# saifahmadgit/go2-sim2real-locomotion-rl

Hardware: AMD Instinct MI355X
Metric: env-steps/sec (all envs) Go2 walk 4096 envs; 1/2/4/8-GPU scaling (higher is better)
Workload: dtype f32

## Files before the change

go2_sim2real_locomotion_rl_amd/csrc/go2sim.hip:

```cpp

#include <hip/hip_runtime.h>

#include <algorithm>
#include <cstddef>
#include <cstdint>
#include <cstdio>
#include <cstdlib>
#include <cstring>
#include <new>
#include <vector>

#include "../../include/go2sim.h"
#include "../../include/go2sim_detmath.h"

#define DEV __device__ __forceinline__
#define DEVN __device__ __noinline__

namespace {

constexpr int NL = GO2SIM_NL, ND = GO2SIM_ND, NQ = GO2SIM_NQ, NG = GO2SIM_NG, NJ = GO2SIM_NJ;
constexpr int NPAIR = GO2SIM_NPAIR_MAX, MAXC = GO2SIM_MAX_CONTACTS, MAXB = GO2SIM_MAX_BROAD, MAXR = GO2SIM_MAX_ROWS;
constexpr int JOINT_FIXED = 0, JOINT_REVOLUTE = 1, JOINT_FREE = 4;
constexpr int GEOM_PLANE = 0, GEOM_SPHERE = 1, GEOM_CYLINDER = 3, GEOM_BOX = 5, GEOM_TERRAIN = 7;
constexpr int TERRAIN_CB = 4;
// ... 851 lines not shown
  xl2 = v2 * iv.z; xl1 = __builtin_fmaf(-lv.z, xl2, v1) * iv.y; xl0 = __builtin_fmaf(-lv.x, xl1, __builtin_fmaf(-lv.y, xl2, v0)) * iv.x;
#pragma unroll
  for (int k = 0; k < 6; ++k) xb[k] = x[k];
}
#endif
struct DynData {
  float cinr_I[NL * 9], cinr_pos[NL * 3], cinr_mass[NL];
  float crb_I[NL * 9], crb_pos[NL * 3], crb_mass[NL];
  float cdof_ang[ND * 3], cdof_vel[ND * 3], cdofd_ang[ND * 3], cdofd_vel[ND * 3];
  float cd_vel[NL * 3], cd_ang[NL * 3], cdd_vel[NL * 3], cdd_ang[NL * 3], cfrc_vel[NL * 3], cfrc_ang[NL * 3];
  float f_ang[ND * 3], f_vel[ND * 3];
  float vel[ND], qf_applied[ND], qf_passive[ND], force[ND], out[ND], Dinv[ND];
  float M[ND * ND], L[ND * ND];
  int ctrl_mode[ND];
};
#if GO2SIM_FAST_ORDER
static_assert(!ARROW_SHAPE || (offsetof(DynData, Dinv) % 8 == 0 && sizeof(DynData) % 8 == 0), "arrow_solve reads DynData::Dinv with 8-byte LDS loads");
#endif

template <int T>
DEV void tk_stage_links(const E& e, KinData* s, int tl) {
  team_for<NL, T>(tl, [&](int i_l) { st3(s->l_pos, i_l, e.l_pos()[i_l]); st4(s->l_quat, i_l, e.l_quat()[i_l]); });
}
template <int T, class MT>
DEV void tk_kinematics(const MT& m, const E& e, KinData* s, int tl, bool force_update_fixed, DynData* dk = nullptr) {
  PH_BEGIN
  const bool legs = (T == 32 || T == 64) && m.leg_form;
  if (legs) {
    const int r = m.leg_root;
    const int rq = m.joints[m.links[r].joint_start].q_start;
    const V3 rpos = v3(s->qpos[rq], s->qpos[rq + 1], s->qpos[rq + 2]);
    Q4 rquat = q4(s->qpos[rq + 3], s->qpos[rq + 4], s->qpos[rq + 5], s->qpos[rq + 6]);
    const float rn = dm_sqrt(norm_sqr(rquat));
    rquat = q4(rquat.w / rn, rquat.x / rn, rquat.y / rn, rquat.z / rn);
    if (tl == 0) {
      const auto& L = m.links[r];
      const int i_j = L.joint_start, ds = m.joints[i_j].dof_start;
      st3(s->xanchor, i_j, rpos);
      st3(s->xaxis, i_j, v3(0, 0, 1));
      gstore(e, FO(dof_pos), ds + 0, rpos.x); gstore(e, FO(dof_pos), ds + 1, rpos.y); gstore(e, FO(dof_pos), ds + 2, rpos.z);
      if (dk) { dk->out[ds] = rpos.x; dk->out[ds + 1] = rpos.y; dk->out[ds + 2] = rpos.z; }
      st3(s->l_pos, r, rpos); st4(s->l_quat, r, rquat); e.l_pos()[r] = rpos; e.l_quat()[r] = rquat;
    }
    Q4 ql = q4(0, 0, 0, 0);
    if (tl < LEG_K * LEG_D) {
      const Joint& J = m.joints[m.links[m.leg_links[tl]].joint_start];
      const float dp = s->qpos[J.q_start] - m.qpos0[J.q_start];
      gstore(e, FO(dof_pos), J.dof_start, dp);
// ... 56 lines not shown
          pos = pos_; quat = quat_;
          gstore(e, FO(dof_pos), dof_start + 0, pos.x); gstore(e, FO(dof_pos), dof_start + 1, pos.y); gstore(e, FO(dof_pos), dof_start + 2, pos.z);
          if (dk) { dk->out[dof_start] = pos.x; dk->out[dof_start + 1] = pos.y; dk->out[dof_start + 2] = pos.z; }
        } else if (J.type == JOINT_REVOLUTE) {
          V3 axis = m.dofs[dof_start].motion_ang;
          V3 anchor = transform_by_quat(J.pos, quat) + pos;
          st3(s->xanchor, i_j, anchor);
          st3(s->xaxis, i_j, transform_by_quat(axis, quat));
          float dp = s->qpos[q_start] - m.qpos0[q_start];
          gstore(e, FO(dof_pos), dof_start, dp);
          if (dk) dk->out[dof_start] = dp;
          Q4 qloc = rotvec_to_quat(axis * dp, m.eps);
          quat = transform_quat_by_quat(qloc, quat);
          pos = anchor - transform_by_quat(J.pos, quat);
        }
      }
      if (!(L.parent == -1 && L.is_fixed)) { st3(s->l_pos, i_l, pos); st4(s->l_quat, i_l, quat); e.l_pos()[i_l] = pos; e.l_quat()[i_l] = quat; }
    }
    team_sync();
  }
  PH(18)
  for (int i_l = tl; i_l < NL; i_l += T) {
    const auto& L = m.links[i_l];
    s->mass[i_l] = L.mass + gload(e, FO(mass_shift), i_l);
    V3 ipbw; Q4 iq;
    transform_pos_quat_by_trans_quat(L.inertial_pos + (V3)e.com_shift()[i_l], L.inertial_quat, ld3(s->l_pos, i_l), ld4(s->l_quat, i_l), ipbw, iq);
    st3(s->i_pos, i_l, ipbw); st4(s->i_quat, i_l, iq);
  }
  team_sync();
  V3 rc[2];
#pragma unroll
  for (int i_e = 0; i_e < 2; ++i_e) {
    const Entity& en = m.entities[i_e];
    V3 root_com_bw = v3(0, 0, 0); float mass_sum = 0.0f;
    for (int i_l = en.link_start; i_l < en.link_end; ++i_l) {
      float mass = s->mass[i_l];
      mass_sum = mass_sum + mass;
      root_com_bw = root_com_bw + mass * ld3(s->i_pos, i_l);
    }
    rc[i_e] = root_com_bw / mass_sum;
  }
  team_sync();
  for (int i_l = tl; i_l < NL; i_l += T) {
    const auto& L = m.links[i_l];
    V3 r = (L.entity == 0) ? rc[0] : rc[1];
    e.root_com()[i_l] = r;
    V3 ip = ld3(s->i_pos, i_l) - r;
    Q4 iq = ld4(s->i_quat, i_l);
    if (!dk) e.i_pos()[i_l] = ip;
// ... 187 lines not shown
    atomicOr(&e.err()[0], GO2SIM_ERR_INVALID_ACC_NAN);
  }
  team_sync();
}

template <int T>
DEV void integrate_fk_body(const Pool& P, const ModelS* __restrict__ mp, int b, KinData* lds, char* ms_raw, bool pre, float pre_vel, float pre_acc) {
  const ModelS& ms = *(const ModelS*)ms_raw;
  wg_dma_to_lds<(int)sizeof(ModelS)>(ms_raw, mp);
  const int tl = threadIdx.x % T, slot = threadIdx.x / T;
  const ModelView m(&ms, mp);
  E e(P, b < P.B ? b : P.B - 1);
  KinData* s = &lds[slot];
  PH_BEGIN
  if (pre) { if (tl < ND) { s->vel[tl] = pre_vel; s->vel_next[tl] = pre_acc; } }
  else {
    team_stage<ND, T>(tl, [&](int d) { return gload(e, FO(vel), d); }, [&](int d, float v) { s->vel[d] = v; });
    team_stage<ND, T>(tl, [&](int d) { return aload(e, AO(acc), d); }, [&](int d, float a) { s->vel_next[d] = a; });
  }
  team_stage<NQ, T>(tl, [&](int q) { return gload(e, FO(qpos), q); }, [&](int q, float v) { s->qpos[q] = v; });
  team_for<ND, T>(tl, [&](int d) { s->vel_next[d] = s->vel[d] + s->vel_next[d] * m.substep_dt; });
  if (tl == 0) s->valid = 1;
  tk_stage_links<T>(e, s, tl);
  team_sync();
  if (b >= P.B) return;
  tk_integrate<T>(m, e, s, tl);
  PH(40)
  tk_kinematics<T>(m, e, s, tl, false);
  PH(41)
}
template <int T>
__global__ __launch_bounds__(64) void k_integrate_fk_team(Pool P, const ModelS* __restrict__ mp) {
  STAMP(STK_INT_FK)
  constexpr int EPW = 64 / T;
  __shared__ KinData lds[EPW];
  __shared__ alignas(16) char ms_raw[MODELS_LDS_BYTES];
  integrate_fk_body<T>(P, mp, xcd_block() * EPW + (int)threadIdx.x / T, lds, ms_raw, false, 0.0f, 0.0f);
}

template <int T>
__global__ __launch_bounds__(64) void k_fk_team(Pool P, const ModelS* __restrict__ mp, int force_update_fixed, const int* __restrict__ cond) {
  constexpr int EPW = 64 / T;
  __shared__ KinData lds[EPW];
  __shared__ alignas(16) char ms_raw[MODELS_LDS_BYTES];
  const ModelS& ms = *(const ModelS*)ms_raw;
  if (cond && *cond <= 0) return;
  wg_dma_to_lds<(int)sizeof(ModelS)>(ms_raw, mp);
  const int tl = threadIdx.x % T, slot = threadIdx.x / T;
  const int b = xcd_block() * EPW + slot;
  const ModelView m(&ms, mp);
  E e(P, b < P.B ? b : P.B - 1);
  KinData* s = &lds[slot];
  team_stage<ND, T>(tl, [&](int d) { return gload(e, FO(vel), d); }, [&](int d, float v) { s->vel[d] = v; });
  team_stage<NQ, T>(tl, [&](int q) { return gload(e, FO(qpos), q); }, [&](int q, float v) { s->qpos[q] = v; });
  tk_stage_links<T>(e, s, tl);
  team_sync();
  if (b >= P.B) return;
  tk_kinematics<T>(m, e, s, tl, force_update_fixed != 0);
}

template <int T, class MT>
DEV void tk_dynamics(const MT& m, const E& e, DynData* s, int tl, bool env_valid) {
  PH_BEGIN
  const bool legs = (T == 32 || T == 64) && m.leg_form;
  if (legs) {
    for (int c = tl; c < 13; c += T) {
      auto at = [&](int i_l) -> float* { return (c < 9) ? &s->crb_I[9 * i_l + c] : ((c < 12) ? &s->crb_pos[3 * i_l + c - 9] : &s->crb_mass[i_l]); };
      const int r = m.leg_root;
      float x[LEG_K][LEG_D];
#pragma unroll
      for (int l = 0; l < LEG_K; ++l)
#pragma unroll
        for (int d = 0; d < LEG_D; ++d) x[l][d] = *at(m.leg_links[LEG_D * l + d]);
      float a = *at(r);
#pragma unroll
      for (int l = 0; l < LEG_K; ++l) {
#pragma unroll
        for (int d = LEG_D - 2; d >= 0; --d) { x[l][d] = x[l][d] + x[l][d + 1]; *at(m.leg_links[LEG_D * l + d]) = x[l][d]; }
      }
#pragma unroll
      for (int l = 0; l < LEG_K; ++l) a = a + x[l][0];
      *at(r) = a;
    }
    team_sync();
  }
// ... 201 lines not shown
  for (int lev = (legs ? -1 : m.n_levels - 2); lev >= 0; --lev) {
    int n_par = m.level_start[lev + 1] - m.level_start[lev];
    for (int w = tl; w < n_par * 6; w += T) {
      int i_p = m.level_links[m.level_start[lev] + w / 6], comp = w % 6;
      float* dst = (comp < 3) ? &s->cfrc_vel[3 * i_p + comp] : &s->cfrc_ang[3 * i_p + comp - 3];
      float a = *dst;
      for (int c = m.child_start[i_p]; c < m.child_start[i_p + 1]; ++c) {
        int i_l = m.child_list[c];
        a = a + ((comp < 3) ? s->cfrc_vel[3 * i_l + comp] : s->cfrc_ang[3 * i_l + comp - 3]);
      }
      *dst = a;
    }
    team_sync();
  }
  for (int i_d = tl; i_d < ND; i_d += T) {
    int i_l = m.dof_link[i_d];
    float qf_bias = dot(ld3(s->cdof_ang, i_d), ld3(s->cfrc_ang, i_l)) + dot(ld3(s->cdof_vel, i_d), ld3(s->cfrc_vel, i_l));
    float f = s->qf_passive[i_d] - qf_bias + s->qf_applied[i_d];
    s->force[i_d] = f;
    if (env_valid) { astore(e, AO(force), i_d, f); astore(e, AO(qf_smooth), i_d, f); }
  }
  team_sync();
  PH(24)
  bool solved = false;
#if GO2SIM_FAST_ORDER
  if constexpr (T == 32 || T == 64) {
    if (arrow) {
      const int leg = (tl >> 3) & 3, u = tl & 7, ub = u < 6 ? u : 5;
      const int p0 = dm_arrow_dof(m.arrow_mode, leg, 0), p1 = dm_arrow_dof(m.arrow_mode, leg, 1), p2 = dm_arrow_dof(m.arrow_mode, leg, 2);
      float xb[6], x0, x1, x2;
      arrow_solve<T>(AF, s->force[p0], s->force[p1], s->force[p2], s->force[ub], s->Dinv, tl, xb, x0, x1, x2);
      if (tl == 0) {
#pragma unroll
        for (int k = 0; k < 6; ++k) s->out[k] = xb[k];
      }
      if (tl < 32 && u == 0) { s->out[p0] = x0; s->out[p1] = x1; s->out[p2] = x2; }
      solved = true;
    }
  }
#endif
  if (!solved) {
    float y[ND];
#pragma unroll
    for (int i_d_ = 0; i_d_ < ND; ++i_d_) {
      const int i_d = ND - i_d_ - 1;
      float cur = s->force[i_d];
// ... 28 lines not shown
}
template <int T>
struct BroadData {
  alignas(16) float amin[NG * 4], amax[NG * 4];
  alignas(16) unsigned long long skey[2 * NG];
  alignas(8) int rank_mm[NG * 2];
  int cand_key[MAXB], cand_pair[MAXB];
  unsigned pair_sorted[MAXB];
};
static_assert(NPAIR <= (1 << 16) && NG <= (1 << 8), "broad_word: 8 bits per geom, 16 bits of pair index");
DEV unsigned broad_word(int packed, int pidx) { return (unsigned)packed | ((unsigned)pidx << 16); }
constexpr int BROAD_PAD = 12;
template <int T> constexpr bool BROAD_OVERLAY = sizeof(BroadData<T>) + BROAD_PAD <= sizeof(DynData);
template <bool OVERLAY, int T> struct BroadSeparate { BroadData<T> k[64 / T]; DEV BroadData<T>* at(int slot, DynData*) { return &k[slot]; } };
template <int T> struct BroadSeparate<true, T> {
  DEV BroadData<T>* at(int slot, DynData* d) {
    static_assert(sizeof(BroadData<T>) + BROAD_PAD <= sizeof(DynData) && sizeof(DynData) % 4 == 0 && alignof(BroadData<T>) == 16, "BroadData overlay");
    return (BroadData<T>*)((char*)d + (16 - (slot * (int)sizeof(DynData)) % 16) % 16);
  }
};
static_assert((BROAD_OVERLAY<16> && BROAD_OVERLAY<32> && BROAD_OVERLAY<64>) || NG != 28 || ND != 18, "the Go2 shape keeps the dynamics kernels' LDS size");

template <int T>
DEV void tk_broadphase(const Model& m, const E& e, BroadData<T>* s, int tl) {
  const float inf = dm_bits2f(0x7f800000u);
  PH_BEGIN
  const int nc_old = e.n_contacts()[0];
  const bool first = e.first_time()[0] != 0;
  const unsigned ncv_old = (unsigned)e.ncache_valid()[tl < NCV ? tl : NCV - 1];
  constexpr int n2 = 2 * NG, NK = (2 * NG + T - 1) / T, NPI = (NPAIR + T - 1) / T, NGR = (NG + T - 1) / T;
  int sig_[NK];
#pragma unroll
  for (int q = 0; q < NK; ++q) { const int i = tl + q * T; sig_[q] = e.sort_ig()[i < n2 ? i : n2 - 1]; }
  int packed_[NPI];
  {
    const int n_pairs = m.n_pairs;
#pragma unroll
    for (int it = 0; it < NPI; ++it) { int pidx = it * T + tl; int v = m.pair_list[pidx < NPAIR ? pidx : NPAIR - 1]; packed_[it] = (pidx < n_pairs) ? v : -1; }
  }
  V3 lower_[NGR], upper_[NGR];
#pragma unroll
  for (int g = 0; g < NGR; ++g) {
    const int i_g = (g * T + tl < NG) ? g * T + tl : NG - 1;
    V3 lower = v3(inf, inf, inf), upper = v3(-inf, -inf, -inf);
    V3 gp = e.g_pos()[i_g]; Q4 gq = e.g_quat()[i_g];
#pragma unroll
    for (int c = 0; c < 8; ++c) {
      V3 corner = transform_by_trans_quat(m.geoms[i_g].aabb[c], gp, gq);
      lower = vmin(lower, corner); upper = vmax(upper, corner);
    }
    lower_[g] = lower; upper_[g] = upper;
  }
  team_sync();
#pragma unroll
  for (int g = 0; g < NGR; ++g) {
    const int i_g = (g * T + tl < NG) ? g * T + tl : NG - 1;
    *(float4*)&s->amin[4 * i_g] = make_float4(lower_[g].x, lower_[g].y, lower_[g].z, 0.0f);
    *(float4*)&s->amax[4 * i_g] = make_float4(upper_[g].x, upper_[g].y, upper_[g].z, 0.0f);
  }
  team_sync();
  PH(30)
  int r[NK]; float sorted_v[NK]; int sorted_sg[NK];
  unsigned long long key[NK];
#pragma unroll
  for (int q = 0; q < NK; ++q) {
    const int i = (tl + q * T < n2) ? tl + q * T : n2 - 1;
    const int sg = first ? ((i >> 1) | ((i & 1) ? 0x100 : 0)) : sig_[q];
    const int g = sg & 0xff;
    const float v = (sg & 0x100) ? s->amax[4 * g] : s->amin[4 * g];
    unsigned u = (unsigned)__float_as_int(v + 0.0f);
    u = (u & 0x80000000u) ? ~u : (u | 0x80000000u);
// ... 83 lines not shown
  const int tl = threadIdx.x % T, slot = threadIdx.x / T;
  const int b = xcd_block() * EPW + slot;
  const bool env_valid = b < P.B;
  const ModelView m(&ms, mp);
  E e(P, env_valid ? b : P.B - 1);
  DynData* s = &lds[slot];
  PH_BEGIN
  team_stage<NL * 9, T>(tl, [&](int k) { return aload(e, AO(cinr_inertial), k); }, [&](int k, float v) { s->cinr_I[k] = v; s->crb_I[k] = v; });
  team_stage<NL * 3, T>(tl, [&](int k) { return aload(e, AO(cinr_pos), k); }, [&](int k, float v) { s->cinr_pos[k] = v; s->crb_pos[k] = v; });
  team_stage<NL, T>(tl, [&](int k) { return aload(e, AO(cinr_mass), k); }, [&](int k, float v) { s->cinr_mass[k] = v; s->crb_mass[k] = v; });
  team_stage<ND, T>(tl, [&](int d) { return __int_as_float((int)e.ctrl_mode()[d]); }, [&](int d, float v) { s->ctrl_mode[d] = __float_as_int(v); });
  team_stage<ND * 3, T>(tl, [&](int k) { return aload(e, AO(cdof_ang), k); }, [&](int k, float v) { s->cdof_ang[k] = v; });
  team_stage<ND * 3, T>(tl, [&](int k) { return aload(e, AO(cdof_vel), k); }, [&](int k, float v) { s->cdof_vel[k] = v; });
  team_stage<ND * 3, T>(tl, [&](int k) { return aload(e, AO(cdofd_ang), k); }, [&](int k, float v) { s->cdofd_ang[k] = v; });
  team_stage<ND * 3, T>(tl, [&](int k) { return aload(e, AO(cdofd_vel), k); }, [&](int k, float v) { s->cdofd_vel[k] = v; });
  team_stage<ND, T>(tl, [&](int d) { return gload(e, FO(ctrl_force), d); }, [&](int d, float v) { s->qf_applied[d] = v; });
  team_stage<ND, T>(tl, [&](int d) { return gload(e, FO(ctrl_pos), d); }, [&](int d, float v) { s->qf_passive[d] = v; });
  team_stage<ND, T>(tl, [&](int d) { return gload(e, FO(ctrl_vel), d); }, [&](int d, float v) { s->force[d] = v; });
  team_stage<ND, T>(tl, [&](int d) { return gload(e, FO(dof_pos), d); }, [&](int d, float v) { s->out[d] = v; });
  team_stage<NL * 6, T>(tl, [&](int k) { return gload(e, FO(ext), k); },
                        [&](int k, float v) { int i_l = k / 6, c = k % 6; if (c < 3) s->cfrc_ang[3 * i_l + c] = v; else s->cfrc_vel[3 * i_l + c - 3] = v; });
  team_sync();
  PH(20)
  tk_dynamics<T>(m, e, s, tl, env_valid);
  if (env_valid) tk_broadphase<T>(*gm, e, lds_b.at(slot, s), tl);
}


template <bool OVERLAY, int EPW> struct KinSeparate { KinData k[EPW]; DEV KinData* at(int slot, void*) { return &k[slot]; } };
template <int EPW> struct KinSeparate<true, EPW> { DEV KinData* at(int, void* overlay) { return (KinData*)overlay; } };
constexpr bool KIN_OVERLAY = sizeof(KinData) <= 2 * sizeof(float) * ND * ND;
template <int T>
DEV void integrate_fk_dynamics_body(const Pool& P, const ModelS* __restrict__ mp, const Model* __restrict__ gm, int b, DynData* lds_d, char* ms_raw,
                                    KinSeparate<KIN_OVERLAY, 64 / T>& lds_k, BroadSeparate<BROAD_OVERLAY<T>, T>& lds_b, bool pre, float pre_vel, float pre_acc) {
  const ModelS& ms = *(const ModelS*)ms_raw;
  wg_dma_to_lds<(int)sizeof(ModelS)>(ms_raw, mp);
  const int tl = threadIdx.x % T, slot = threadIdx.x / T;
  const ModelView m(&ms, mp);
  asm volatile("" : "+v"(b));
  E e(P, b < P.B ? b : P.B - 1);
  DynData* d = &lds_d[slot];
  static_assert(offsetof(DynData, L) == offsetof(DynData, M) + sizeof(float) * ND * ND, "KinData overlay");
  KinData* s = lds_k.at(slot, d->M);
  PH_BEGIN
  if (pre) { if (tl < ND) { s->vel[tl] = pre_vel; s->vel_next[tl] = pre_acc; } }
  else {
    team_stage<ND, T>(tl, [&](int i) { return gload(e, FO(vel), i); }, [&](int i, float v) { s->vel[i] = v; });
    team_stage<ND, T>(tl, [&](int i) { return aload(e, AO(acc), i); }, [&](int i, float a) { s->vel_next[i] = a; });
  }
  team_stage<NQ, T>(tl, [&](int q) { return gload(e, FO(qpos), q); }, [&](int q, float v) { s->qpos[q] = v; });
  team_stage<ND, T>(tl, [&](int i) { return __int_as_float((int)e.ctrl_mode()[i]); }, [&](int i, float v) { d->ctrl_mode[i] = __float_as_int(v); });
  team_stage<ND, T>(tl, [&](int i) { return gload(e, FO(ctrl_force), i); }, [&](int i, float v) { d->qf_applied[i] = v; });
  team_stage<ND, T>(tl, [&](int i) { return gload(e, FO(ctrl_pos), i); }, [&](int i, float v) { d->qf_passive[i] = v; });
  team_stage<ND, T>(tl, [&](int i) { return gload(e, FO(ctrl_vel), i); }, [&](int i, float v) { d->force[i] = v; });
  team_stage<NL * 6, T>(tl, [&](int k) { return gload(e, FO(ext), k); },
                        [&](int k, float v) { int i_l = k / 6, c = k % 6; if (c < 3) d->cfrc_ang[3 * i_l + c] = v; else d->cfrc_vel[3 * i_l + c - 3] = v; });
  team_for<ND, T>(tl, [&](int i) { s->vel_next[i] = s->vel[i] + s->vel_next[i] * m.substep_dt; });
  if (tl == 0) s->valid = 1;
  tk_stage_links<T>(e, s, tl);
  team_sync();
  if (b >= P.B) return;
  tk_integrate<T>(m, e, s, tl);
  PH(40)
  tk_kinematics<T>(m, e, s, tl, false, d);
  team_for<ND, T>(tl, [&](int i) { d->vel[i] = s->vel[i]; });
  team_sync();
  PH(41)
  tk_dynamics<T>(m, e, d, tl, true);
  tk_broadphase<T>(*gm, e, lds_b.at(slot, d), tl);
}
template <int T>
__global__ __launch_bounds__(64) void k_integrate_fk_dynamics_team(Pool P, const ModelS* __restrict__ mp, const Model* __restrict__ gm) {
  STAMP(STK_INT_FK_DYN)
  constexpr int EPW = 64 / T;
  __shared__ alignas(16) DynData lds_d[EPW];
  __shared__ alignas(16) char ms_raw[MODELS_LDS_BYTES];
  __shared__ KinSeparate<KIN_OVERLAY, EPW> lds_k;
  __shared__ BroadSeparate<BROAD_OVERLAY<T>, T> lds_b;
  integrate_fk_dynamics_body<T>(P, mp, gm, xcd_block() * EPW + (int)threadIdx.x / T, lds_d, ms_raw, lds_k, lds_b, false, 0.0f, 0.0f);
}

DEV int wrap180(float x) {
  if (!(x >= 0.0f)) return 0;
  int i = (x >= 180.0f) ? (int)(x - 180.0f) : (int)x;
  return (i > 179) ? 179 : i;
}
DEV int clampidx(float x) {
  if (!(x >= 0.0f)) return 0;
  return (x >= 179.0f) ? 179 : (int)x;
}
DEV V3 support_cylinder_local(const Model& m, const Geom& G, V3 d_mesh, int* vid_out = nullptr) {
  const float PI = 3.14159265358979323846f;
// ... 1906 lines not shown
        const float active = (float)(rw.Ja < 0.0f);
        const float xs[3] = {rw.q0 * active, rw.q1 * active, rw.q2 * active}, bs[3] = {t0, t1, t2};
        float tot[3];
        team_serial_sum<T, 3>(xs, bs, tl, nseg, tot);
        t0 = tot[0]; t1 = tot[1]; t2 = tot[2];
        done = true;
      }
    }
    if (!done) {
#pragma unroll 16
      for (int c = 0; c < n_con; ++c) {
        float active = (float)(s->Jaref[c] < 0.0f);
        t0 = t0 + s->qf0[c] * active; t1 = t1 + s->qf1[c] * active; t2 = t2 + s->qf2[c] * active;
      }
    }
    p0.alpha = 0.0f; p0.cost = t0; p0.grad = t1; p0.hess = 2.0f * t2;
    if (p0.hess <= 0.0f) p0.hess = m.eps;
  }
  LS_MARK(50)
  return ts_linesearch_tail<T>(m, s, tl, n_con, nseg, rw, gtol, qg0, qg1, qg2, p0);
}

#undef LS_MARK
template <int T, class S, class MT>
DEV int ts_solve(const MT& m, const E& e, S* s, int tl, int nc, int n_con, unsigned lim_mask, int ws_flag) {
  PH_BEGIN
  const bool ws = (n_con > 0) && ws_flag;
  team_stage<NTRI, T>(tl, [&](int k) { return aload(e, AO(mass_mat), k); }, [&](int k, float v) { int i, j; tri_index(m, k, i, j); s->M[i * DS + j] = v; s->M[j * DS + i] = v; });
  team_stage<ND * 3, T>(tl, [&](int k) { return aload(e, AO(cdof_ang), k); }, [&](int k, float v) { s->cdof_ang[k] = v; });
  team_stage<ND * 3, T>(tl, [&](int k) { return aload(e, AO(cdof_vel), k); }, [&](int k, float v) { s->cdof_vel[k] = v; });
  team_stage<NL * 3, T>(tl, [&](int k) { return gload(e, FO(root_com), k); }, [&](int k, float v) { s->root_com[k] = v; });
  team_stage<ND, T>(tl, [&](int d) { return gload(e, FO(vel), d); }, [&](int d, float v) { s->vel[d] = v; });
  team_stage<ND, T>(tl, [&](int d) { return aload(e, AO(force), d); }, [&](int d, float v) { s->force[d] = v; });
  team_stage<ND, T>(tl, [&](int d) { return aload(e, AO(acc_smooth), d); }, [&](int d, float v) { s->acc_smooth[d] = v; });
  team_stage<ND, T>(tl, [&](int d) { return aload(e, AO(qacc_ws), d); }, [&](int d, float v) { s->qacc[d] = v; });
  team_sync();
  if (!ws) team_for<ND, T>(tl, [&](int d) { s->qacc[d] = s->acc_smooth[d]; });
  team_sync();
  PH(0)
  bool rows_coupled = false;
  for (int r = tl; r < 4 * nc; r += T) {
    int i_col = r >> 2, i = r & 3;
    int link_a = e.c_link()[i_col], link_b = e.c_link()[MAXC + i_col];
    V3 cpos = e.c_pos()[i_col], cnormal = e.c_normal()[i_col];
    float friction = e.c_friction()[i_col], pen = e.c_pen()[i_col];
    float sol[7];
    auto csol = e.c_sol()[i_col];
#pragma unroll
    for (int k = 0; k < 7; ++k) sol[k] = csol[k];
    V3 d1, d2;
    orthogonals(cnormal, d1, d2);
    float invweight = m.links[link_a].invweight[0];
    if (link_b > -1) invweight = invweight + m.links[link_b].invweight[0];
    V3 d = (float)(2 * (i % 2) - 1) * ((i < 2) ? d1 : d2);
    V3 n = d * friction - cnormal;
    float* row = &s->J[r * DS];
#pragma unroll
    for (int i_d = 0; i_d < DS; ++i_d) row[i_d] = 0.0f;
    float jac_qvel = 0.0f;
    unsigned legs = 0u;
    for (int i_ab = 0; i_ab < 2; ++i_ab) {
      float sign = -1.0f; int link = link_a;
      if (i_ab == 1) { sign = 1.0f; link = link_b; }
      while (link > -1) {
        V3 t_pos = cpos - v3(s->root_com[3 * link], s->root_com[3 * link + 1], s->root_com[3 * link + 2]);
        const int nd = m.links[link].n_dofs, de = m.links[link].dof_end;
        if (nd > 0 && de > 6) legs |= 1u << dm_arrow_leg(m.arrow_mode, de - 1);
        for (int i_d_ = 0; i_d_ < nd; ++i_d_) {
          int i_d = de - 1 - i_d_;
          V3 ca = v3(s->cdof_ang[3 * i_d], s->cdof_ang[3 * i_d + 1], s->cdof_ang[3 * i_d + 2]);
          V3 cv = v3(s->cdof_vel[3 * i_d], s->cdof_vel[3 * i_d + 1], s->cdof_vel[3 * i_d + 2]);
          V3 velv = cv - cross(t_pos, ca);
          V3 diff = sign * velv;
          float j = dot(diff, n);
          jac_qvel = jac_qvel + j * s->vel[i_d];
          row[i_d] = row[i_d] + j;
        }
        link = m.links[link].parent;
      }
    }
    float imp, aref;
    imp_aref(sol, -pen, jac_qvel, -pen, imp, aref);
    float diag = invweight + friction * friction * invweight;
    diag *= 2.0f * friction * friction * (1.0f - imp) / imp;
    diag = fmx(diag, m.eps);
    s->aref[r] = aref; s->efc_D[r] = 1.0f / diag;
    rows_coupled = rows_coupled || (legs & (legs - 1u)) != 0u;
  }
  for (int i_j = tl; i_j < NJ; i_j += T) {
    if (!((lim_mask >> i_j) & 1u)) continue;
    const Joint& Jt = m.joints[i_j];
    int i_d = Jt.dof_start;
    float q = gload(e, FO(qpos), Jt.q_start);
    float pos_delta_min = q - m.dofs[i_d].limit[0];
    float pos_delta_max = m.dofs[i_d].limit[1] - q;
    float pos_delta = fmn(pos_delta_min, pos_delta_max);
    {
      int r = 4 * nc + __popc(lim_mask & ((1u << i_j) - 1u));
      float j = (float)((pos_delta_min < pos_delta_max) * 2 - 1);
      float jac_qvel = j * s->vel[i_d];
      float imp, aref;
      imp_aref(Jt.sol_params, pos_delta, jac_qvel, pos_delta, imp, aref);
      float diag = fmx(m.dofs[i_d].invweight * (1.0f - imp) / imp, m.eps);
      s->aref[r] = aref; s->efc_D[r] = 1.0f / diag;
      float* row = &s->J[r * DS];
#pragma unroll
      for (int i_d2 = 0; i_d2 < DS; ++i_d2) row[i_d2] = 0.0f;
      row[i_d] = j;
    }
  }
  team_sync();
  PH(1)
  {
    float qa[ND];
#pragma unroll
    for (int d = 0; d < ND; ++d) qa[d] = s->qacc[d];
// ... 123 lines not shown
      f = f + n * s->efc_force[i_c * 4 + i_dir];
    }
    e.c_force()[i_c] = f;
    cf[4 * i_c] = f.x; cf[4 * i_c + 1] = f.y; cf[4 * i_c + 2] = f.z;
    ((int*)cf)[4 * i_c + 3] = pre ? lk0 : (e.c_link()[i_c] | (e.c_link()[MAXC + i_c] << 8));
  }
  team_sync();
  for (int i_l = tl; i_l < NL; i_l += T) {
    V3 acc = v3(0, 0, 0);
#pragma unroll 4
    for (int i_c = 0; i_c < nc; ++i_c) {
      int lk = ((const int*)cf)[4 * i_c + 3];
      int la = lk & 0xff, lb = lk >> 8;
      V3 f = v3(cf[4 * i_c], cf[4 * i_c + 1], cf[4 * i_c + 2]);
      if (la == i_l) acc = acc - f;
      if (lb == i_l) acc = acc + f;
    }
    e.contact_force()[i_l] = acc;
  }
}

template <int T>
DEVN void ts_solve_overflow(float* Pf, int* Pi, int PB, float* Pfa, int* Pia, int b, const LinkS* lnk, const unsigned char* tri_i, const unsigned char* tri_j,
                            const Model* __restrict__ gm, SolverData<MAXR>* s, int tl, int nc, int n_con, unsigned lim_mask, int ws_flag) {
  Pool P; P.f = Pf; P.i = Pi; P.B = PB; P.fa = Pfa; P.ia = Pia;
  const E e(P, b);
  const ModelView m(lnk, tri_i, tri_j, gm);
  int iters = ts_solve<T>(m, e, s, tl, nc, n_con, lim_mask, ws_flag);
  ts_commit<T>(m, e, s, tl, nc, n_con, iters);
}

template <int T, int RLN>
DEV void solve_body(const Pool& P, const Model* __restrict__ gm, const ModelS* __restrict__ mp, SolverData<MAXR>* __restrict__ overflow,
                    const int* __restrict__ lpt_rec, int* __restrict__ lpt_next, int lpt_cap, SolverData<RLN>* lds, char* blk_raw, int& b_out, bool& resident_out) {
  constexpr int EPW = 64 / T;
  const LinkS* lnk = (const LinkS*)blk_raw;
  const unsigned char* tri_i = (const unsigned char*)(blk_raw + sizeof(LinkS) * NL);
  const unsigned char* tri_j = tri_i + (NTRI + 1);
  static_assert(T >= NJ, "one lane per joint in the limit test");
  PH_BEGIN
  wg_dma_to_lds<SOLVER_BLOCK_BYTES>(blk_raw, mp->links);
  const int tl = threadIdx.x % T, slot = threadIdx.x / T;
  const int b = lpt_take(lpt_rec, lpt_cap, P.B, EPW, slot);
  if (lpt_next && blockIdx.x == 0) for (int i = threadIdx.x; i < 8 * LPT_CLS; i += 64) lpt_next[i] = 0;
  const bool env_valid = b < P.B;
  b_out = b; resident_out = false;
  E e(P, env_valid ? b : P.B - 1);
  const int nc = e.n_contacts()[0];
  const int ws_flag = e.is_warmstart()[0];
  const JLim jl = mp->jlim[tl < NJ ? tl : NJ - 1];
  const float q_lim = gload(e, FO(qpos), jl.q_start < 0 ? 0 : jl.q_start);
  const bool lim = tl < NJ && jl.q_start >= 0 && fmn(q_lim - jl.lo, jl.hi - q_lim) < 0;
  const unsigned lim_mask = (unsigned)((__ballot(lim) >> (slot * T)) & ((T == 64) ? ~0ull : ((1ull << T) - 1ull)));
  const int n_lim = __popc(lim_mask);
  __syncthreads();
  PH(9)
  const ModelView m(lnk, tri_i, tri_j, gm);
  if (!env_valid) return;
  const int n_con = 4 * nc + n_lim;
  if (n_con <= RLN) {
    SolverData<RLN>* s = &lds[slot];
    resident_out = true;
    int iters = ts_solve<T>(m, e, s, tl, nc, n_con, lim_mask, ws_flag);
    PH(10)
    ts_commit<T>(m, e, s, tl, nc, n_con, iters);
    PH(11)
  } else {
    ts_solve_overflow<T>(P.f, P.i, P.B, P.fa, P.ia, b, lnk, tri_i, tri_j, gm, &overflow[b], tl, nc, n_con, lim_mask, ws_flag);
  }
}
template <int T, int RLN>
__global__ __launch_bounds__(64) __attribute__((amdgpu_waves_per_eu(2, 2))) void k_constraint_solve_team(Pool P, const Model* __restrict__ gm, const ModelS* __restrict__ mp, SolverData<MAXR>* __restrict__ overflow,
                                                                                                         const int* __restrict__ lpt_rec, int* __restrict__ lpt_next, int lpt_cap) {
  STAMP(STK_SOLVE)
  constexpr int EPW = 64 / T;
  __shared__ SolverData<RLN> lds[EPW];
  __shared__ alignas(16) char blk_raw[lds_dma_bytes(SOLVER_BLOCK_BYTES)];
  int b; bool resident;
  solve_body<T, RLN>(P, gm, mp, overflow, lpt_rec, lpt_next, lpt_cap, lds, blk_raw, b, resident);
}

constexpr size_t cmax(size_t a, size_t b) { return a > b ? a : b; }
template <int T, int RLN, bool WITH_DYN>
__global__ __launch_bounds__(64) __attribute__((amdgpu_waves_per_eu(2, 2))) void k_solve_integrate_team(Pool P, const Model* __restrict__ gm, const ModelS* __restrict__ mp,
                                                                                                        SolverData<MAXR>* __restrict__ overflow, const int* __restrict__ lpt_rec,
                                                                                                        int* __restrict__ lpt_next, int lpt_cap) {
  STAMP(STK_SOLVE)
  constexpr int EPW = 64 / T;
  constexpr size_t SOLVE_OFF = (sizeof(SolverData<RLN>) * EPW + 15) / 16 * 16, DYN_OFF = (sizeof(DynData) * EPW + 15) / 16 * 16, KIN_OFF = (sizeof(KinData) * EPW + 15) / 16 * 16;
  constexpr size_t SOLVE_BYTES = SOLVE_OFF + lds_dma_bytes(SOLVER_BLOCK_BYTES);
  constexpr size_t KSEP_OFF = (sizeof(KinSeparate<KIN_OVERLAY, EPW>) + 15) / 16 * 16;
// ... 461 lines not shown
      } else {
        if (g.push_counter % g.push_interval == 0) {
          dm_u4 r = rng4(seed, RNG_PUSH, b, step_count, 0);
          psf_[0] = rand_float(g.push_force_lo, g.push_force_hi, r.v[0]);
          psf_[1] = rand_float(g.push_force_lo, g.push_force_hi, r.v[1]);
          psf_[2] = 0.0f;
          psf[0] = psf_[0]; psf[1] = psf_[1]; psf[2] = psf_[2];
          rem0 = rand_int(c.i[GO2SIM_IC_PUSH_DUR_LO], c.i[GO2SIM_IC_PUSH_DUR_HI], r.v[2]);
        }
        const float active = (rem0 > 0) ? 1.0f : 0.0f;
        const V3 force = v3(psf_[0] * active, psf_[1] * active, psf_[2] * active);
        cpf[0] = force.x; cpf[1] = force.y; cpf[2] = force.z;
        prem[0] = imx(rem0 - 1, 0);
        const V3 tq = cross(pl_pos - pl_com, force);
        const float x0 = ext_[0] - tq.x, x1 = ext_[1] - tq.y, x2 = ext_[2] - tq.z, x3 = ext_[3] - force.x, x4 = ext_[4] - force.y, x5 = ext_[5] - force.z;
        ext[6 * pl + 0] = x0; ext[6 * pl + 1] = x1; ext[6 * pl + 2] = x2; ext[6 * pl + 3] = x3; ext[6 * pl + 4] = x4; ext[6 * pl + 5] = x5;
        s->cfrc_ang[3 * pl + 0] = x0; s->cfrc_ang[3 * pl + 1] = x1; s->cfrc_ang[3 * pl + 2] = x2;
        s->cfrc_vel[3 * pl + 0] = x3; s->cfrc_vel[3 * pl + 1] = x4; s->cfrc_vel[3 * pl + 2] = x5;
      }
    }
  }
  team_sync();
  PH(20)
  tk_dynamics<T>(m, e, s, tl, env_valid);
  if (env_valid) tk_broadphase<T>(*gm, e, lds_b.at(slot, s), tl);
}

struct RewCtx { float link_vel_xy[8], foot_z[4], foot_xy[8]; float vel_world[3]; int was_reset; };
struct RewState {
  float cmd[3], blv[3], bav[3], pg[3], base_pos[3];
  float dof_pos[NM], dof_vel[NM], last_dof_vel[NM], target[NM], ctrl_force[NM];
  float actions[NA], last_actions[NA];
  float fat[4]; int fc[4];
  float last_x;
  float ctrl_pos[NM], ctrl_vel[NM], s_vel[NM], s_dof_pos[NM]; int ctrl_mode[NM];
};
DEV void load_rew_state(const DCfg& c, const E& e, RewState& rs) {
  auto cmd = e.commands(); auto ldv = e.last_dof_vel(); auto t = e.target_dof_pos(); auto cf = e.ctrl_force(); auto a = e.actions(); auto la = e.last_actions();
  auto fat = e.feet_air_time();
#pragma unroll
  for (int i = 0; i < 3; ++i) rs.cmd[i] = cmd[i];
#pragma unroll
  for (int i = 0; i < NM; ++i) { rs.last_dof_vel[i] = ldv[i]; rs.target[i] = t[i]; rs.ctrl_force[i] = cf[c.i[GO2SIM_IC_MOTOR_DOF0 + i]]; }
#pragma unroll
  for (int i = 0; i < NA; ++i) { rs.actions[i] = a[i]; rs.last_actions[i] = la[i]; }
#pragma unroll
  for (int i = 0; i < 4; ++i) rs.fat[i] = fat[i];
  rs.last_x = e.last_base_pos_x()[0];
// ... 743 lines not shown
                                                        float* __restrict__ timeout_out) {
  STAMP(STK_POST_B)
  constexpr int EPW = 64 / T;
  __shared__ KinData fk_lds[EPW];
  __shared__ alignas(16) char ms_raw[MODELS_LDS_BYTES];
  const bool fk_needed = gp->n_reset_now > 0;
  const int na = cp->i[GO2SIM_IC_NUM_ACTIONS], nobs = cp->i[GO2SIM_IC_NUM_OBS], npriv = cp->i[GO2SIM_IC_NUM_PRIV_OBS], env_kind = cp->i[GO2SIM_IC_ENV_KIND];
  const int lane = (int)threadIdx.x & 63, wave = (int)threadIdx.x >> 6;
  if (wave == 1) {
    if (!fk_needed) return;
    wg_dma_to_lds<(int)sizeof(ModelS)>(ms_raw, msp, lane);
  }
  const int tl = lane % T, slot = lane / T;
  const int b = xcd_block() * EPW + slot;
  if (wave == 1) {
    __syncthreads();
    __builtin_amdgcn_fence(__ATOMIC_ACQUIRE, "workgroup");
    if (b >= P.B) return;
    E e(P, b);
    KinData* ks = &fk_lds[slot];
    team_stage<ND, T>(tl, [&](int d) { return gload(e, FO(vel), d); }, [&](int d, float v) { ks->vel[d] = v; });
    team_stage<NQ, T>(tl, [&](int q) { return gload(e, FO(qpos), q); }, [&](int q, float v) { ks->qpos[q] = v; });
    tk_stage_links<T>(e, ks, tl);
    team_sync();
    const ModelView mv((const ModelS*)ms_raw, msp);
    tk_kinematics<T>(mv, e, ks, tl, true);
    return;
  }
  const bool valid = b < P.B;
  PH_BEGIN
  const Model& m = *mp; const DCfg& c = *cp; const Glob& g = *gp;
  E e(P, valid ? b : P.B - 1);
  auto fk_refresh = [&]() {};
  const int was_reset = valid ? e.reset_buf()[0] : 0;
  if (valid && g.n_reset_now > 0) {
    {
      const ResetDraws rd = env_reset_draws_team<T>(c, g, e, b, seed, tl, was_reset != 0);
      if (tl == 0 && was_reset) env_reset_one(m, c, g, e, b, seed, &rd);
    }
    const bool per_env = c.i[GO2SIM_IC_PER_ENV_GLOBAL_DR] != 0;
    if (c.i[GO2SIM_IC_HAS_FRICTION_DR] && !per_env) for (int i = tl; i < NG; i += T) e.geom_friction()[i] = g.friction;
    if (tl == 0) {
      int bl = c.i[GO2SIM_IC_BASE_LINK];
      if (c.i[GO2SIM_IC_HAS_MASS_DR] && !per_env) e.mass_shift()[bl] = g.mass_shift;
      if (c.i[GO2SIM_IC_HAS_COM_DR]) e.com_shift()[bl] = v3(g.com_shift[0], g.com_shift[1], g.com_shift[2]);
      if (c.i[GO2SIM_IC_HAS_LEGM_DR]) for (int k = 0; k < 4; ++k) e.mass_shift()[c.i[GO2SIM_IC_HIP_LINK0 + k]] = g.leg_mass_shift[k];
    }
    team_sync();
  }
// ... 1185 lines not shown
```

Measured before the change: 18.20 million.

## Prefetch global loads into registers ahead of kinematics, broadphase and solver

Moves global-memory loads earlier so they overlap with other work. Per-link mass/COM shifts are loaded before the staging sync, broadphase geom poses and AABB corners are issued mid-dynamics through a callback, and solver inputs (mass matrix, cdof, velocities, first contact record, joint qpos) are loaded into registers before the solve and then written to LDS. It also uses asm barriers to keep the compiler from sinking these loads. The aim is to hide global load latency, at the cost of more live registers and possible lower occupancy or spills.

```diff
diff --git a/go2_sim2real_locomotion_rl_amd/csrc/go2sim.hip b/go2_sim2real_locomotion_rl_amd/csrc/go2sim.hip
--- a/go2_sim2real_locomotion_rl_amd/csrc/go2sim.hip
+++ b/go2_sim2real_locomotion_rl_amd/csrc/go2sim.hip
@@ -897,8 +897,16 @@
 DEV void tk_stage_links(const E& e, KinData* s, int tl) {
   team_for<NL, T>(tl, [&](int i_l) { st3(s->l_pos, i_l, e.l_pos()[i_l]); st4(s->l_quat, i_l, e.l_quat()[i_l]); });
 }
+struct KinDR { float mass_shift; V3 com_shift; };
+template <int T>
+DEV KinDR tk_load_dr(const E& e, int tl) {
+  static_assert(T >= NL, "link tl is the lane's only link in the COM pass");
+  const int i_l = tl < NL ? tl : NL - 1;
+  KinDR dr; dr.mass_shift = gload(e, FO(mass_shift), i_l); dr.com_shift = e.com_shift()[i_l];
+  return dr;
+}
 template <int T, class MT>
-DEV void tk_kinematics(const MT& m, const E& e, KinData* s, int tl, bool force_update_fixed, DynData* dk = nullptr) {
+DEV void tk_kinematics(const MT& m, const E& e, KinData* s, int tl, bool force_update_fixed, const KinDR& dr, DynData* dk = nullptr) {
   PH_BEGIN
   const bool legs = (T == 32 || T == 64) && m.leg_form;
   if (legs) {
@@ -1001,9 +1009,9 @@
   PH(18)
   for (int i_l = tl; i_l < NL; i_l += T) {
     const auto& L = m.links[i_l];
-    s->mass[i_l] = L.mass + gload(e, FO(mass_shift), i_l);
+    s->mass[i_l] = L.mass + dr.mass_shift;
     V3 ipbw; Q4 iq;
-    transform_pos_quat_by_trans_quat(L.inertial_pos + (V3)e.com_shift()[i_l], L.inertial_quat, ld3(s->l_pos, i_l), ld4(s->l_quat, i_l), ipbw, iq);
+    transform_pos_quat_by_trans_quat(L.inertial_pos + dr.com_shift, L.inertial_quat, ld3(s->l_pos, i_l), ld4(s->l_quat, i_l), ipbw, iq);
     st3(s->i_pos, i_l, ipbw); st4(s->i_quat, i_l, iq);
   }
   team_sync();
@@ -1237,11 +1245,12 @@
   team_for<ND, T>(tl, [&](int d) { s->vel_next[d] = s->vel[d] + s->vel_next[d] * m.substep_dt; });
   if (tl == 0) s->valid = 1;
   tk_stage_links<T>(e, s, tl);
+  const KinDR dr = tk_load_dr<T>(e, tl);
   team_sync();
   if (b >= P.B) return;
   tk_integrate<T>(m, e, s, tl);
   PH(40)
-  tk_kinematics<T>(m, e, s, tl, false);
+  tk_kinematics<T>(m, e, s, tl, false, dr);
   PH(41)
 }
 template <int T>
@@ -1269,13 +1278,14 @@
   team_stage<ND, T>(tl, [&](int d) { return gload(e, FO(vel), d); }, [&](int d, float v) { s->vel[d] = v; });
   team_stage<NQ, T>(tl, [&](int q) { return gload(e, FO(qpos), q); }, [&](int q, float v) { s->qpos[q] = v; });
   tk_stage_links<T>(e, s, tl);
+  const KinDR dr = tk_load_dr<T>(e, tl);
   team_sync();
   if (b >= P.B) return;
-  tk_kinematics<T>(m, e, s, tl, force_update_fixed != 0);
-}
-
-template <int T, class MT>
-DEV void tk_dynamics(const MT& m, const E& e, DynData* s, int tl, bool env_valid) {
+  tk_kinematics<T>(m, e, s, tl, force_update_fixed != 0, dr);
+}
+
+template <int T, class MT, class F>
+DEV void tk_dynamics(const MT& m, const E& e, DynData* s, int tl, bool env_valid, F issue_next) {
   PH_BEGIN
   const bool legs = (T == 32 || T == 64) && m.leg_form;
   if (legs) {
@@ -1523,6 +1533,7 @@
   }
   team_sync();
   PH(24)
+  issue_next();
   bool solved = false;
 #if GO2SIM_FAST_ORDER
   if constexpr (T == 32 || T == 64) {
@@ -1597,13 +1608,28 @@
 static_assert((BROAD_OVERLAY<16> && BROAD_OVERLAY<32> && BROAD_OVERLAY<64>) || NG != 28 || ND != 18, "the Go2 shape keeps the dynamics kernels' LDS size");
 
 template <int T>
-DEV void tk_broadphase(const Model& m, const E& e, BroadData<T>* s, int tl) {
+struct BroadOps {
+  static constexpr int NK = (2 * NG + T - 1) / T, NPI = (NPAIR + T - 1) / T, NGR = (NG + T - 1) / T;
+  V3 gp[NGR]; Q4 gq[NGR]; V3 corner[NGR][8];
+};
+template <int T>
+DEV void tk_broadphase_issue(const Model& m, const E& e, int tl, BroadOps<T>& o) {
+#pragma unroll
+  for (int g = 0; g < BroadOps<T>::NGR; ++g) {
+    const int i_g = (g * T + tl < NG) ? g * T + tl : NG - 1;
+    o.gp[g] = e.g_pos()[i_g]; o.gq[g] = e.g_quat()[i_g];
+#pragma unroll
+    for (int c = 0; c < 8; ++c) o.corner[g][c] = m.geoms[i_g].aabb[c];
+  }
+}
+template <int T>
+DEV void tk_broadphase(const Model& m, const E& e, BroadData<T>* s, int tl, const BroadOps<T>& o) {
   const float inf = dm_bits2f(0x7f800000u);
   PH_BEGIN
   const int nc_old = e.n_contacts()[0];
   const bool first = e.first_time()[0] != 0;
   const unsigned ncv_old = (unsigned)e.ncache_valid()[tl < NCV ? tl : NCV - 1];
-  constexpr int n2 = 2 * NG, NK = (2 * NG + T - 1) / T, NPI = (NPAIR + T - 1) / T, NGR = (NG + T - 1) / T;
+  constexpr int n2 = 2 * NG, NK = BroadOps<T>::NK, NPI = BroadOps<T>::NPI, NGR = BroadOps<T>::NGR;
   int sig_[NK];
 #pragma unroll
   for (int q = 0; q < NK; ++q) { const int i = tl + q * T; sig_[q] = e.sort_ig()[i < n2 ? i : n2 - 1]; }
@@ -1616,12 +1642,11 @@
   V3 lower_[NGR], upper_[NGR];
 #pragma unroll
   for (int g = 0; g < NGR; ++g) {
-    const int i_g = (g * T + tl < NG) ? g * T + tl : NG - 1;
     V3 lower = v3(inf, inf, inf), upper = v3(-inf, -inf, -inf);
-    V3 gp = e.g_pos()[i_g]; Q4 gq = e.g_quat()[i_g];
+    const V3 gp = o.gp[g]; const Q4 gq = o.gq[g];
 #pragma unroll
     for (int c = 0; c < 8; ++c) {
-      V3 corner = transform_by_trans_quat(m.geoms[i_g].aabb[c], gp, gq);
+      V3 corner = transform_by_trans_quat(o.corner[g][c], gp, gq);
       lower = vmin(lower, corner); upper = vmax(upper, corner);
     }
     lower_[g] = lower; upper_[g] = upper;
@@ -1751,8 +1776,9 @@
                         [&](int k, float v) { int i_l = k / 6, c = k % 6; if (c < 3) s->cfrc_ang[3 * i_l + c] = v; else s->cfrc_vel[3 * i_l + c - 3] = v; });
   team_sync();
   PH(20)
-  tk_dynamics<T>(m, e, s, tl, env_valid);
-  if (env_valid) tk_broadphase<T>(*gm, e, lds_b.at(slot, s), tl);
+  BroadOps<T> bo;
+  tk_dynamics<T>(m, e, s, tl, env_valid, [&]() { tk_broadphase_issue<T>(*gm, e, tl, bo); });
+  if (env_valid) tk_broadphase<T>(*gm, e, lds_b.at(slot, s), tl, bo);
 }
 
 
@@ -1787,16 +1813,18 @@
   team_for<ND, T>(tl, [&](int i) { s->vel_next[i] = s->vel[i] + s->vel_next[i] * m.substep_dt; });
   if (tl == 0) s->valid = 1;
   tk_stage_links<T>(e, s, tl);
+  const KinDR dr = tk_load_dr<T>(e, tl);
   team_sync();
   if (b >= P.B) return;
   tk_integrate<T>(m, e, s, tl);
   PH(40)
-  tk_kinematics<T>(m, e, s, tl, false, d);
+  tk_kinematics<T>(m, e, s, tl, false, dr, d);
   team_for<ND, T>(tl, [&](int i) { d->vel[i] = s->vel[i]; });
   team_sync();
   PH(41)
-  tk_dynamics<T>(m, e, d, tl, true);
-  tk_broadphase<T>(*gm, e, lds_b.at(slot, d), tl);
+  BroadOps<T> bo;
+  tk_dynamics<T>(m, e, d, tl, true, [&]() { tk_broadphase_issue<T>(*gm, e, tl, bo); });
+  tk_broadphase<T>(*gm, e, lds_b.at(slot, d), tl, bo);
 }
 template <int T>
 __global__ __launch_bounds__(64) void k_integrate_fk_dynamics_team(Pool P, const ModelS* __restrict__ mp, const Model* __restrict__ gm) {
@@ -3749,32 +3777,68 @@
 }
 
 #undef LS_MARK
+template <int N, int T> struct StageRegs { float v[(N + T - 1) / T]; };
+template <int N, int T, class FL>
+DEV void stage_ld(StageRegs<N, T>& r, int tl, FL ld) {
+#pragma unroll
+  for (int q = 0; q < (N + T - 1) / T; ++q) { const int k = q * T + tl; r.v[q] = ld(k < N ? k : N - 1); }
+}
+template <int N, int T, class FS>
+DEV void stage_st(const StageRegs<N, T>& r, int tl, FS st) {
+#pragma unroll
+  for (int q = 0; q < (N + T - 1) / T; ++q) { const int k = q * T + tl; st(k < N ? k : N - 1, r.v[q]); }
+}
+template <int T>
+struct SolveOps {
+  StageRegs<NTRI, T> M; StageRegs<ND * 3, T> cdof_ang, cdof_vel; StageRegs<NL * 3, T> root_com; StageRegs<ND, T> vel, force, acc_smooth, qacc_ws;
+};
+template <int T>
+DEV void solve_ops_load(const E& e, int tl, SolveOps<T>& o) {
+  stage_ld(o.M, tl, [&](int k) { return aload(e, AO(mass_mat), k); });
+  stage_ld(o.cdof_ang, tl, [&](int k) { return aload(e, AO(cdof_ang), k); });
+  stage_ld(o.cdof_vel, tl, [&](int k) { return aload(e, AO(cdof_vel), k); });
+  stage_ld(o.root_com, tl, [&](int k) { return gload(e, FO(root_com), k); });
+  stage_ld(o.vel, tl, [&](int d) { return gload(e, FO(vel), d); });
+  stage_ld(o.force, tl, [&](int d) { return aload(e, AO(force), d); });
+  stage_ld(o.acc_smooth, tl, [&](int d) { return aload(e, AO(acc_smooth), d); });
+  stage_ld(o.qacc_ws, tl, [&](int d) { return aload(e, AO(qacc_ws), d); });
+}
+struct ContactRec { int link_a, link_b; V3 pos, normal; float friction, pen, sol[7]; };
+static_assert(MAXC >= 16, "the prefetched contact record (lane tl: contact tl >> 2) lies inside the env's record at every team size");
+DEV ContactRec contact_rec_load(const E& e, int i_col) {
+  ContactRec c;
+  c.link_a = e.c_link()[i_col]; c.link_b = e.c_link()[MAXC + i_col];
+  c.pos = e.c_pos()[i_col]; c.normal = e.c_normal()[i_col];
+  c.friction = e.c_friction()[i_col]; c.pen = e.c_pen()[i_col];
+  auto csol = e.c_sol()[i_col];
+#pragma unroll
+  for (int k = 0; k < 7; ++k) c.sol[k] = csol[k];
+  return c;
+}
+
 template <int T, class S, class MT>
-DEV int ts_solve(const MT& m, const E& e, S* s, int tl, int nc, int n_con, unsigned lim_mask, int ws_flag) {
+DEV int ts_solve(const MT& m, const E& e, S* s, int tl, int nc, int n_con, unsigned lim_mask, int ws_flag, const SolveOps<T>& ops, const ContactRec& rec0, float q_lim) {
   PH_BEGIN
   const bool ws = (n_con > 0) && ws_flag;
-  team_stage<NTRI, T>(tl, [&](int k) { return aload(e, AO(mass_mat), k); }, [&](int k, float v) { int i, j; tri_index(m, k, i, j); s->M[i * DS + j] = v; s->M[j * DS + i] = v; });
-  team_stage<ND * 3, T>(tl, [&](int k) { return aload(e, AO(cdof_ang), k); }, [&](int k, float v) { s->cdof_ang[k] = v; });
-  team_stage<ND * 3, T>(tl, [&](int k) { return aload(e, AO(cdof_vel), k); }, [&](int k, float v) { s->cdof_vel[k] = v; });
-  team_stage<NL * 3, T>(tl, [&](int k) { return gload(e, FO(root_com), k); }, [&](int k, float v) { s->root_com[k] = v; });
-  team_stage<ND, T>(tl, [&](int d) { return gload(e, FO(vel), d); }, [&](int d, float v) { s->vel[d] = v; });
-  team_stage<ND, T>(tl, [&](int d) { return aload(e, AO(force), d); }, [&](int d, float v) { s->force[d] = v; });
-  team_stage<ND, T>(tl, [&](int d) { return aload(e, AO(acc_smooth), d); }, [&](int d, float v) { s->acc_smooth[d] = v; });
-  team_stage<ND, T>(tl, [&](int d) { return aload(e, AO(qacc_ws), d); }, [&](int d, float v) { s->qacc[d] = v; });
+  stage_st(ops.M, tl, [&](int k, float v) { int i, j; tri_index(m, k, i, j); s->M[i * DS + j] = v; s->M[j * DS + i] = v; });
+  stage_st(ops.cdof_ang, tl, [&](int k, float v) { s->cdof_ang[k] = v; });
+  stage_st(ops.cdof_vel, tl, [&](int k, float v) { s->cdof_vel[k] = v; });
+  stage_st(ops.root_com, tl, [&](int k, float v) { s->root_com[k] = v; });
+  stage_st(ops.vel, tl, [&](int d, float v) { s->vel[d] = v; });
+  stage_st(ops.force, tl, [&](int d, float v) { s->force[d] = v; });
+  stage_st(ops.acc_smooth, tl, [&](int d, float v) { s->acc_smooth[d] = v; });
+  stage_st(ops.qacc_ws, tl, [&](int d, float v) { s->qacc[d] = v; });
   team_sync();
   if (!ws) team_for<ND, T>(tl, [&](int d) { s->qacc[d] = s->acc_smooth[d]; });
   team_sync();
   PH(0)
   bool rows_coupled = false;
-  for (int r = tl; r < 4 * nc; r += T) {
-    int i_col = r >> 2, i = r & 3;
-    int link_a = e.c_link()[i_col], link_b = e.c_link()[MAXC + i_col];
-    V3 cpos = e.c_pos()[i_col], cnormal = e.c_normal()[i_col];
-    float friction = e.c_friction()[i_col], pen = e.c_pen()[i_col];
-    float sol[7];
-    auto csol = e.c_sol()[i_col];
-#pragma unroll
-    for (int k = 0; k < 7; ++k) sol[k] = csol[k];
+  auto contact_row = [&](const int r, const ContactRec& cr) {
+    const int i = r & 3;
+    const int link_a = cr.link_a, link_b = cr.link_b;
+    const V3 cpos = cr.pos, cnormal = cr.normal;
+    const float friction = cr.friction, pen = cr.pen;
+    const float (&sol)[7] = cr.sol;
     V3 d1, d2;
     orthogonals(cnormal, d1, d2);
     float invweight = m.links[link_a].invweight[0];
@@ -3813,12 +3877,15 @@
     diag = fmx(diag, m.eps);
     s->aref[r] = aref; s->efc_D[r] = 1.0f / diag;
     rows_coupled = rows_coupled || (legs & (legs - 1u)) != 0u;
-  }
+  };
+  if (tl < 4 * nc) contact_row(tl, rec0);
+  for (int r = tl + T; r < 4 * nc; r += T) contact_row(r, contact_rec_load(e, r >> 2));
+  static_assert(T >= NJ, "joint tl is the lane's only joint: q_lim is its coordinate");
   for (int i_j = tl; i_j < NJ; i_j += T) {
     if (!((lim_mask >> i_j) & 1u)) continue;
     const Joint& Jt = m.joints[i_j];
     int i_d = Jt.dof_start;
-    float q = gload(e, FO(qpos), Jt.q_start);
+    float q = q_lim;
     float pos_delta_min = q - m.dofs[i_d].limit[0];
     float pos_delta_max = m.dofs[i_d].limit[1] - q;
     float pos_delta = fmn(pos_delta_min, pos_delta_max);
@@ -3988,11 +4055,14 @@
 
 template <int T>
 DEVN void ts_solve_overflow(float* Pf, int* Pi, int PB, float* Pfa, int* Pia, int b, const LinkS* lnk, const unsigned char* tri_i, const unsigned char* tri_j,
-                            const Model* __restrict__ gm, SolverData<MAXR>* s, int tl, int nc, int n_con, unsigned lim_mask, int ws_flag) {
+                            const Model* __restrict__ gm, SolverData<MAXR>* s, int tl, int nc, int n_con, unsigned lim_mask, int ws_flag, float q_lim) {
   Pool P; P.f = Pf; P.i = Pi; P.B = PB; P.fa = Pfa; P.ia = Pia;
   const E e(P, b);
   const ModelView m(lnk, tri_i, tri_j, gm);
-  int iters = ts_solve<T>(m, e, s, tl, nc, n_con, lim_mask, ws_flag);
+  SolveOps<T> ops;
+  solve_ops_load<T>(e, tl, ops);
+  const ContactRec rec0 = contact_rec_load(e, tl >> 2);
+  int iters = ts_solve<T>(m, e, s, tl, nc, n_con, lim_mask, ws_flag, ops, rec0, q_lim);
   ts_commit<T>(m, e, s, tl, nc, n_con, iters);
 }
 
@@ -4012,10 +4082,22 @@
   const bool env_valid = b < P.B;
   b_out = b; resident_out = false;
   E e(P, env_valid ? b : P.B - 1);
-  const int nc = e.n_contacts()[0];
-  const int ws_flag = e.is_warmstart()[0];
-  const JLim jl = mp->jlim[tl < NJ ? tl : NJ - 1];
-  const float q_lim = gload(e, FO(qpos), jl.q_start < 0 ? 0 : jl.q_start);
+  int b_pre = env_valid ? b : P.B - 1, tl_pre = tl;
+  asm volatile("" : "+v"(b_pre), "+v"(tl_pre));
+  const E e_pre(P, b_pre);
+  const JLim jl = mp->jlim[tl_pre < NJ ? tl_pre : NJ - 1];
+  const int nc = e_pre.n_contacts()[0];
+  const int ws_flag = e_pre.is_warmstart()[0];
+  SolveOps<T> ops;
+  solve_ops_load<T>(e_pre, tl_pre, ops);
+  const ContactRec rec0 = contact_rec_load(e_pre, tl_pre >> 2);
+  float q_team[(NQ + T - 1) / T];
+#pragma unroll
+  for (int q = 0; q < (NQ + T - 1) / T; ++q) { const int k = q * T + tl_pre; q_team[q] = gload(e_pre, FO(qpos), k < NQ ? k : NQ - 1); }
+  const int q_idx = jl.q_start < 0 ? 0 : jl.q_start;
+  float q_lim = __shfl(q_team[0], q_idx % T, T);
+#pragma unroll
+  for (int q = 1; q < (NQ + T - 1) / T; ++q) { const float v = __shfl(q_team[q], q_idx % T, T); if (q_idx / T == q) q_lim = v; }
   const bool lim = tl < NJ && jl.q_start >= 0 && fmn(q_lim - jl.lo, jl.hi - q_lim) < 0;
   const unsigned lim_mask = (unsigned)((__ballot(lim) >> (slot * T)) & ((T == 64) ? ~0ull : ((1ull << T) - 1ull)));
   const int n_lim = __popc(lim_mask);
@@ -4027,12 +4109,15 @@
   if (n_con <= RLN) {
     SolverData<RLN>* s = &lds[slot];
     resident_out = true;
-    int iters = ts_solve<T>(m, e, s, tl, nc, n_con, lim_mask, ws_flag);
+    int iters = ts_solve<T>(m, e, s, tl, nc, n_con, lim_mask, ws_flag, ops, rec0, q_lim);
     PH(10)
-    ts_commit<T>(m, e, s, tl, nc, n_con, iters);
+    int b_com = b;
+    asm volatile("" : "+v"(b_com));
+    const E e_com(P, b_com);
+    ts_commit<T>(m, e_com, s, tl, nc, n_con, iters);
     PH(11)
   } else {
-    ts_solve_overflow<T>(P.f, P.i, P.B, P.fa, P.ia, b, lnk, tri_i, tri_j, gm, &overflow[b], tl, nc, n_con, lim_mask, ws_flag);
+    ts_solve_overflow<T>(P.f, P.i, P.B, P.fa, P.ia, b, lnk, tri_i, tri_j, gm, &overflow[b], tl, nc, n_con, lim_mask, ws_flag, q_lim);
   }
 }
 template <int T, int RLN>
@@ -4540,8 +4625,9 @@
   }
   team_sync();
   PH(20)
-  tk_dynamics<T>(m, e, s, tl, env_valid);
-  if (env_valid) tk_broadphase<T>(*gm, e, lds_b.at(slot, s), tl);
+  BroadOps<T> bo;
+  tk_dynamics<T>(m, e, s, tl, env_valid, [&]() { tk_broadphase_issue<T>(*gm, e, tl, bo); });
+  if (env_valid) tk_broadphase<T>(*gm, e, lds_b.at(slot, s), tl, bo);
 }
 
 struct RewCtx { float link_vel_xy[8], foot_z[4], foot_xy[8]; float vel_world[3]; int was_reset; };
@@ -5331,9 +5417,10 @@
     team_stage<ND, T>(tl, [&](int d) { return gload(e, FO(vel), d); }, [&](int d, float v) { ks->vel[d] = v; });
     team_stage<NQ, T>(tl, [&](int q) { return gload(e, FO(qpos), q); }, [&](int q, float v) { ks->qpos[q] = v; });
     tk_stage_links<T>(e, ks, tl);
+    const KinDR dr = tk_load_dr<T>(e, tl);
     team_sync();
     const ModelView mv((const ModelS*)ms_raw, msp);
-    tk_kinematics<T>(mv, e, ks, tl, true);
+    tk_kinematics<T>(mv, e, ks, tl, true, dr);
     return;
   }
   const bool valid = b < P.B;
```

After: 18.02 million. No clear change (-1.0%).
